# RunhuiWang/DeltaPQ

Hardware: AMD Instinct MI355X
Metric: queries/sec, SIFT1M-shaped m=8 k=256 topk=100 (higher is better)
Workload: dtype f64 sum of f32 table entries (u8 code decode; the reference's incremental f64 stack); 1 GPU

## Files before the change

deltapq_amd/_lib.py:

```python
import ctypes
import os

_HERE = os.path.dirname(os.path.abspath(__file__))
LIB_PATH = os.environ.get("DPQ_LIB_PATH") or os.path.join(_HERE, "csrc", "libdeltapq_amd.so")

c_i32, c_i64, c_f32 = ctypes.c_int32, ctypes.c_int64, ctypes.c_float
P = ctypes.POINTER


class OpenOpts(ctypes.Structure):
    _fields_ = [("device", c_i32), ("shard_rank", c_i32), ("shard_count", c_i32), ("chunks_per_segment", c_i32),
                ("cand_capacity", c_i32), ("num_codes", c_i32), ("bootstrap", c_i32), ("batch_decode", c_i32),
                ("global_offset", c_i64), ("global_n_codes", c_i64),
                ("stream_max_queries", c_i32), ("coarse_below", c_i32), ("plan_ratios", c_i32 * 3), ("boot_cap", c_i32),
                ("boot_target", c_i32), ("flags", c_i32), ("batch_tile_nodes", c_i64)]


class Info(ctypes.Structure):
    _fields_ = [("n_codes_total", c_i64), ("n_bytes_total", c_i64), ("node_lo", c_i64), ("node_hi", c_i64),
                ("algorithmic_bytes", c_i64), ("device_bytes", c_i64), ("n_diffs", c_i64), ("M", c_i32),
                ("K", c_i32), ("Ds", c_i32), ("n_segments", c_i32), ("chunks_per_segment", c_i32),
                ("max_depth", c_i32), ("device", c_i32), ("cand_capacity", c_i32), ("bootstrap_bytes", c_i64),
                ("bootstrap_stride", c_i32), ("batch_decode_mb", c_i32), ("strand_bytes", c_i64)]

# ... 212 lines not shown
    ("dpq_opq_train", ctypes.c_int,
     [_VP, c_i64, ctypes.c_int, ctypes.c_int, ctypes.c_int, P(OpqOpts), _VP, _VP, P(OpqStats)]),
    ("dpq_write_rotation", ctypes.c_int, [ctypes.c_char_p, _VP, ctypes.c_int]),
    ("dpq_read_rotation", ctypes.c_int, [ctypes.c_char_p, P(c_i32), _VP]),
    ("dpq_query_batch_tables", ctypes.c_int, [_VP, _VP, _VP, ctypes.c_int, ctypes.c_int, _VP, _VP]),
    ("dpq_query_batch_device_tables", ctypes.c_int, [_VP, _VP, _VP, ctypes.c_int, ctypes.c_int, _VP, _VP, _VP]),
    ("dpq_range_search_tables", ctypes.c_int, [_VP, _VP, ctypes.c_int, _VP, P(_VP)]),
    ("dpq_ip_tables", ctypes.c_int, [_VP, _VP, ctypes.c_int, _VP, _VP]),
    ("dpq_ip_tables_device", ctypes.c_int, [_VP, _VP, ctypes.c_int, _VP, _VP, _VP]),
    ("dpq_query_batch_ip", ctypes.c_int, [_VP, _VP, _VP, ctypes.c_int, ctypes.c_int, _VP, _VP, _VP, _VP]),
    ("dpq_query_batch_device_ip", ctypes.c_int, [_VP, _VP, _VP, ctypes.c_int, ctypes.c_int, _VP, _VP, _VP, _VP, _VP]),
    ("dpq_ip_scores", ctypes.c_int, [_VP, _VP, _VP, ctypes.c_int, ctypes.c_int, _VP]),
    ("dpq_profile_enable", ctypes.c_int, [_VP, ctypes.c_int]),
    ("dpq_profile_reset", ctypes.c_int, [_VP]),
    ("dpq_profile_read", ctypes.c_int, [_VP, P(Profile)]),
    ("dpq_debug_scan_time", ctypes.c_int, [_VP, ctypes.c_int, ctypes.c_int, ctypes.c_int, ctypes.c_int, P(ctypes.c_float)]),
    ("dpq_debug_scan_stamps", ctypes.c_int, [_VP, ctypes.c_int, ctypes.c_int, P(ctypes.c_ulonglong), ctypes.c_int, P(ctypes.c_float)]),
    ("dpq_debug_boot_stamps", ctypes.c_int, [_VP, ctypes.c_int, P(ctypes.c_double)]),
    ("dpq_debug_select_time", ctypes.c_int, [_VP, ctypes.c_int, ctypes.c_int, ctypes.c_int, ctypes.c_int, P(ctypes.c_float)]),
    ("dpq_debug_strand1_stamps", ctypes.c_int, [_VP, _VP, ctypes.c_int]),
    ("dpq_debug_range_keys", ctypes.c_int, [_VP, P(c_i64)]),
    ("dpq_debug_filter_tables", ctypes.c_int, [_VP, ctypes.c_int, _VP, c_i64]),
    ("dpq_debug_relabel", ctypes.c_int, [_VP, _VP, ctypes.c_int]),
]

_lib = None
_hip_runtime = None


def _bind_hip_runtime():
    global _hip_runtime
    if _hip_runtime is not None:
        return _hip_runtime
    import importlib.util
    candidates = []
    override = os.environ.get("DPQ_HIP_RUNTIME")
    if override:
        candidates.append(override)
    try:
        spec = importlib.util.find_spec("torch")
        if spec is not None and spec.submodule_search_locations:
            candidates.append(os.path.join(list(spec.submodule_search_locations)[0], "lib", "libamdhip64.so"))
    except (ImportError, ValueError):
        pass
    rocm = os.environ.get("ROCM_PATH", "/opt/rocm")
    candidates += [os.path.join(rocm, "lib", "libamdhip64.so"), "libamdhip64.so"]
# ... 43 lines not shown
```

deltapq_amd/csrc/dpq_capi.cpp:

```cpp
#include "dpq_capi_internal.h"

namespace {

thread_local std::string g_last_error;

}

int fail(int code, const std::string& msg) {
    g_last_error = msg;
    return code;
}

uint64_t next_index_serial() {
    static std::atomic<uint64_t> next{1};
    return next++;
}

bool dev_mode() {
    const char* dev = getenv("DPQ_DEV");
    return dev && atoi(dev) != 0;
}

namespace {

// ... 320 lines not shown
int prepare_batch(dpq_index* x, Batch* b) {
    int rc;
    if ((rc = ensure_plan(x, b->top_k, b->cap, b->plan_shape))) return rc;
    int64_t stride = b->top_k;
    for (size_t l = 1; l < x->level_cnt.size(); ++l)
        stride = std::max(stride, regions_for(x, x->level_cnt[l], b->ngroups, b->top_k, b->cap).stride);
    const int s1_region_cap = std::min(std::max(64, b->top_k), 256);
    if (b->strand1) stride = std::max<int64_t>(stride, (int64_t)b->top_k + (int64_t)dpq::kStrand1Regions * s1_region_cap);
    if (stride > INT32_MAX) return fail(DPQ_ERR_NOMEM, "candidate buffer too large");
    if ((rc = ensure_workspace(x, b->nqp, (int)stride))) return rc;
    b->stride = x->ws().cap;
    if (b->scratch && (rc = ensure_batch_raw(x))) return rc;
    return DPQ_OK;
}

int build_tables(dpq_index* x, const Batch& b, const TableSource& src, hipStream_t stream, bool row_stats = true) {
    Workspace& w = x->ws();
    int rc;
    if (b.one_tile && (rc = ensure_plain_image(x, stream))) return rc;
    {
        Timer t(x, stream, 0);
        const uint8_t* relabel = b.scratch ? x->d_relabel.get() : nullptr;
        uint32_t* tight = x->tune.tighten ? w.d_tight.get() : nullptr;
        if (src.d_tables)
            DPQ_HIP(dpq::launch_tables_ingest(src.d_tables, b.nq, b.nqp, x->M, x->K, w.d_lut32, w.d_lut_min, w.d_overflow,
                                              relabel, w.d_lut32r, tight, src.d_bad, stream));
        else
            DPQ_HIP(dpq::launch_lut_build(x->d_codebook, src.d_queries, b.nq, b.nqp, x->M, x->K, x->Ds, w.d_lut32,
                                          w.d_lut_min, nullptr, w.d_overflow, relabel, w.d_lut32r, tight, stream));
        if (row_stats) DPQ_HIP(dpq::launch_row_stats(w.d_lut32, b.nq, x->M, w.d_lut_stat, stream));
    }
    if (x->prof) x->prof_acc.lut_launches++;
    return DPQ_OK;
}

dpq::ScanArgs batch_scan_args(const dpq_index* x, const Batch& b) {
    const Workspace& w = x->ws();
    dpq::ScanArgs sa{};
    sa.img = x->img;
    if (b.one_tile) sa.img.raw = x->d_plain_image;
    sa.fp32_accum = x->plain ? 1 : 0;
    sa.lut32 = b.labelled ? w.d_lut32r.get() : w.d_lut32.get();
    sa.lut_min = w.d_lut_min;
    sa.lut_stat = w.d_lut_stat;
    sa.thr_key = w.d_thr_key;
    sa.slot_query = nullptr;
    sa.n_queries = b.nq;
    sa.cand_count = w.d_cand_count;
    sa.cand_key = w.d_cand_key;
    sa.cand_stride = b.stride;
    sa.region_off = b.top_k;
    sa.counters = x->prof && !x->prof_scan_only ? x->d_counters.get() : nullptr;
    sa.qtab = w.d_qtab;
// ... 1524 lines not shown
```

deltapq_amd/csrc/dpq_capi_debug.cpp:

```cpp
#include "dpq_capi_internal.h"

namespace {

dpq::ScanArgs debug_scan_args(const dpq_index* x, int nq, int* splits) {
    const Workspace& w = x->ws();
    const int QG = dpq::queries_per_group(x->M);
    dpq::ScanArgs sa{};
    sa.img = x->img;
    sa.fp32_accum = x->plain ? 1 : 0;
    sa.lut32 = w.d_lut32;
    sa.lut_min = w.d_lut_min;
    sa.lut_stat = w.d_lut_stat;
    sa.thr_key = w.d_thr_key;
    sa.slot_query = nullptr;
    sa.n_queries = nq;
    sa.seg_list = nullptr;
    sa.n_seg_pass = x->img.n_segments;
    if (const char* e = getenv("DPQ_DEBUG_NSEG")) sa.n_seg_pass = std::min(x->img.n_segments, atoi(e));
    if (*splits <= 0) *splits = splits_for(sa.n_seg_pass, (nq + QG - 1) / QG);
    sa.cand_count = w.d_cand_count;
    sa.cand_key = w.d_cand_key;
    sa.cand_stride = w.cap;
    sa.region_off = 0;
    sa.region_cap = std::max(1, w.cap / *splits);
// ... 225 lines not shown
        sa.lut_min = w.d_lut_min;
        sa.lut_stat = w.d_lut_stat;
        sa.thr_key = w.d_dbg_thr;
        sa.n_queries = w.dbg_qtab_nq;
        DPQ_HIP(dpq::launch_saturation_debug(sa, slots, d_rec, nullptr));
        DPQ_HIP(hipMemcpy(static_cast<char*>(out) + tables, d_rec.get(), records, hipMemcpyDeviceToHost));
    }
    return DPQ_OK;
    });
}

int dpq_debug_relabel(dpq_index* x, unsigned char* out, int bytes) {
    return guarded([&]() -> int {
    DPQ_DEV_ONLY();
    if (!x || !out || bytes < x->M * 256) return fail(DPQ_ERR_ARG, "bad argument");
    if (!x->d_relabel) return fail(DPQ_ERR_STATE, "the handle has no label map");
    DPQ_HIP(hipSetDevice(x->device));
    DPQ_HIP(hipDeviceSynchronize());
    DPQ_HIP(hipMemcpy(out, x->d_relabel.get(), (size_t)x->M * 256, hipMemcpyDeviceToHost));
    return DPQ_OK;
    });
}

int dpq_debug_range_keys(dpq_index* x, int64_t* max_keys) {
    DPQ_DEV_ONLY();
    if (!x || !max_keys) return fail(DPQ_ERR_ARG, "NULL argument");
    *max_keys = x->range.last_max_keys;
    return DPQ_OK;
}

int dpq_debug_select_time(dpq_index* x, int nq, int top_k, int flags, int reps, float* ms_out) {
    return guarded([&]() -> int {
    DPQ_DEV_ONLY();
    if (!x || !ms_out || !x->ws().d_lut32 || !x->d_l0_id) return fail(DPQ_ERR_STATE, "run a query batch first");
    DPQ_HIP(hipSetDevice(x->device));
    const Workspace& w = x->ws();
    dpq::SelectArgs se{};
    se.shared_id = x->d_l0_id;
    se.shared_code = x->d_l0_code;
    se.shared_n = x->l0_segments * dpq::kChunk * x->img.chunks_per_segment;
    se.cand_count = w.d_cand_count;
    se.cand_key = w.d_cand_key;
    se.cand_stride = w.cap;
    se.region_off = top_k;
    se.scratch = w.d_scratch;
    se.lut32 = w.d_lut32;
// ... 25 lines not shown
```

deltapq_amd/csrc/dpq_kernels.h:

```cpp
#pragma once
#include <hip/hip_runtime.h>

#include <cstdint>

#include "dpq_format.h"

#ifndef DPQ_UNDER_SCAN_PRIO
#define DPQ_UNDER_SCAN_PRIO 3
#endif

namespace dpq {

constexpr int kScanThreads = 1024;
constexpr int kScanWaves = kScanThreads / 64;
constexpr int kMaxTopK = 2048;
constexpr int kSelectThreads = 512;
constexpr int kMaxSplits = 256;
constexpr int kRegionStride = 1 + kMaxSplits;
constexpr int kLevel0Nodes = 3840;
constexpr int kSortMax = 4096;
constexpr int queries_per_group(int M) { return M <= 8 ? 64 : 32; }
constexpr int kTightBuckets = 8;
constexpr int kTightSplits = 32;
constexpr int kTightWords = kTightSplits * kTightBuckets / 4;
constexpr int kS1Replicas = 8, kS1ReplicaWords = 512;
constexpr int kS1HistWords = kS1Replicas * kS1ReplicaWords;
static_assert(queries_per_group(8) * kTightWords >= kS1HistWords, "strand1's histogram exceeds what one query group clears");
constexpr int kLutQueries = 8;
constexpr int kLutMinParts = 4;

struct DeviceImage {
    const uint8_t* nib = nullptr;
    const uint8_t* par = nullptr;
    const uint8_t* carry = nullptr;
    const uint8_t* mask = nullptr;
    const uint8_t* delta = nullptr;
    const uint64_t* seg_delta_off = nullptr;
    const uint8_t* seg_ckpt = nullptr;
    const uint8_t* raw = nullptr;
    const uint64_t* st_ckpt = nullptr;
    const uint32_t* st_mask = nullptr;
    const uint16_t* st_depth = nullptr;
    const uint32_t* st_pbase = nullptr;
    const uint8_t* st_delta = nullptr;
    int32_t n_strips = 0;
    int64_t n_local = 0;
    int64_t n_codes_total = 0;
    uint32_t id_base = 0;
    int32_t n_segments = 0;
    int32_t chunks_per_segment = 4;
    int32_t M = 8, K = 256;
};
// ... 90 lines not shown
    const int32_t* slot_query;
    const uint32_t* cand_count;
    int32_t n_slots, n_regions, n_queries;
    uint32_t* max_count;
    int64_t* lims;
};

struct RangeEmitArgs {
    const int64_t* out_off;
    const uint32_t* cand_count;
    const uint64_t* cand_key;
    int64_t cand_stride;
    int32_t region_off, region_cap, n_regions;
    int32_t lds_keys;
    int32_t* out_ids;
    float* out_dists;
    int64_t out_n;
    uint64_t* scratch;
    int64_t n_codes_total;
};

hipError_t launch_lut_build(const float* d_codebook, const float* d_queries, int nq, int n_slots, int M, int K, int Ds,
                            float* d_lut32, float* d_lut_min, uint32_t* d_cand_count, uint32_t* d_overflow,
                            const uint8_t* d_relabel, float* d_lut_labels, uint32_t* d_tight_hist,
                            hipStream_t stream);
hipError_t launch_decode_list(const DeviceImage& img, const uint32_t* seg_list, int n_seg, const uint8_t* relabel,
                              uint32_t* out_code, hipStream_t stream);
hipError_t launch_decode_segments(const DeviceImage& img, const uint32_t* seg_list, int n_seg, uint32_t* out_id,
                                  uint32_t* out_code, hipStream_t stream);
hipError_t launch_stream(const ScanArgs& a, int n_slots, hipStream_t stream);
hipError_t launch_strand(const ScanArgs& a, int n_slots, hipStream_t stream);
int stream_queries_per_pass(int M, int n_slots);
hipError_t launch_strand1(const ScanArgs& a, int n_slots, hipStream_t stream);
int strand1_workgroups(int n_strips);
constexpr int kStrand1Regions = 256;
hipError_t launch_quantise(const ScanArgs& a, int n_slot_groups, hipStream_t stream);
hipError_t launch_row_stats(const float* d_lut32, int nq, int M, float* d_lut_stat, hipStream_t stream);
hipError_t launch_scan(const ScanArgs& a, int n_slot_groups, int splits, hipStream_t stream);
size_t qtab_bytes_per_group(int M);
hipError_t launch_saturation_debug(const ScanArgs& a, int n_slots, unsigned char* d_out, hipStream_t stream);
int scan_stamp_count();
hipError_t launch_select(const SelectArgs& a, int M, int n_slots, hipStream_t stream);
hipError_t launch_bootstrap(const BootArgs& a, int M, int n_slots, hipStream_t stream);
hipError_t launch_range_count(const RangeCountArgs& a, hipStream_t stream);
hipError_t launch_range_emit(const RangeEmitArgs& a, int n_slots, hipStream_t stream);
hipError_t launch_merge(const int32_t* d_ids, const float* d_dists, int n_lists, int nq, int top_k, int row_stride,
                        int32_t* d_out_ids, float* d_out_dists, hipStream_t stream);
// ... 7 lines not shown
```

deltapq_amd/csrc/dpq_kernels.hip:

```cpp
#include "dpq_kernels.h"
#include "dpq_wave_decoder.h"

#include <atomic>
#include <type_traits>
#include <cfloat>
#include <cmath>

namespace dpq {

static hipError_t ensure_dynamic_lds(const void* fn, size_t bytes, std::atomic<bool>* done);


__device__ __forceinline__ uint32_t and_or(uint32_t a, uint32_t mask, uint32_t c) {
    uint32_t r;
    asm("v_and_or_b32 %0, %1, %2, %3" : "=v"(r) : "v"(a), "s"(mask), "v"(c));
    return r;
}

__device__ __forceinline__ uint64_t make_key(float d, uint32_t id) {
    return ((uint64_t)__float_as_uint(d) << 32) | (uint64_t)id;
}

__device__ __forceinline__ float lut_min_of(const float* __restrict__ lut_min, size_t q, int M, int m) {
    const float4 p = *reinterpret_cast<const float4*>(lut_min + (q * M + m) * kLutMinParts);
    return fminf(fminf(p.x, p.y), fminf(p.z, p.w));
}

__global__ __launch_bounds__(256) void lut_build_kernel(const float* __restrict__ codebook,
                                                         const float* __restrict__ queries, int nq, int n_slots, int M,
                                                         int K, int Ds, float* __restrict__ lut,
                                                         float* __restrict__ lut_min, uint32_t* __restrict__ cand_count,
                                                         uint32_t* __restrict__ overflow, const uint8_t* __restrict__ relabel,
                                                         float* __restrict__ lut_labels, uint32_t* __restrict__ tight_hist) {
    __builtin_amdgcn_s_setprio(DPQ_UNDER_SCAN_PRIO);
    const int q0 = blockIdx.x * kLutQueries, m = blockIdx.y, k = threadIdx.x;
    if (m == 0 && k < kLutQueries && q0 + k < n_slots) {
        if (cand_count) cand_count[q0 + k] = 0;
        if (overflow) overflow[q0 + k] = 0;
    }
    if (m == 0 && tight_hist)
        for (int i = k; i < kLutQueries * kTightWords; i += 256)
            if (q0 * kTightWords + i < n_slots * kTightWords) tight_hist[(size_t)q0 * kTightWords + i] = 0;
    if (q0 >= nq) return;
    float acc[kLutQueries];
#pragma unroll
    for (int j = 0; j < kLutQueries; ++j) acc[j] = 0.0f;
    if (k < K) {
        const float* c = codebook + ((size_t)m * K + k) * Ds;
        const float* qv = queries + (size_t)q0 * M * Ds + (size_t)m * Ds;
        const size_t qstride = (size_t)M * Ds;
        auto step = [&](float& a, float cv, float qd) {
            const float diff = __fsub_rn(cv, qd);
            const double sq = __dmul_rn((double)diff, (double)diff);
            a = (float)__dadd_rn((double)a, sq);
        };
        if ((Ds & 3) == 0) {
            const float4* c4 = reinterpret_cast<const float4*>(c);
            for (int d = 0; d < Ds; d += 4) {
                const float4 v = c4[d >> 2];
#pragma unroll
                for (int j = 0; j < kLutQueries; ++j) {
                    const float* qj = qv + (size_t)min(j, nq - 1 - q0) * qstride + d;
                    step(acc[j], v.x, qj[0]);
                    step(acc[j], v.y, qj[1]);
                    step(acc[j], v.z, qj[2]);
                    step(acc[j], v.w, qj[3]);
                }
            }
        } else {
            for (int d = 0; d < Ds; ++d) {
                const float cv = c[d];
#pragma unroll
                for (int j = 0; j < kLutQueries; ++j) step(acc[j], cv, qv[(size_t)min(j, nq - 1 - q0) * qstride + d]);
            }
        }
    } else {
#pragma unroll
        for (int j = 0; j < kLutQueries; ++j) acc[j] = INFINITY;
    }
#pragma unroll
    for (int j = 0; j < kLutQueries; ++j) {
        if (q0 + j < nq) lut[((size_t)(q0 + j) * M + m) * 256 + k] = acc[j];
        if (lut_labels && q0 + j < nq) lut_labels[((size_t)(q0 + j) * M + m) * 256 + relabel[m * 256 + k]] = acc[j];
        uint32_t v = __float_as_uint(acc[j]);
#pragma unroll
        for (int o = 32; o > 0; o >>= 1) v = min(v, (uint32_t)__shfl_xor((int)v, o));
        if ((k & 63) == 0 && q0 + j < nq) lut_min[((size_t)(q0 + j) * M + m) * kLutMinParts + (k >> 6)] = __uint_as_float(v);
    }
}

template <int M>
__global__ __launch_bounds__(64) void decode_segments_kernel(const DeviceImage img,
                                                              const uint32_t* __restrict__ seg_list,
                                                              uint32_t* __restrict__ out_id,
                                                              uint32_t* __restrict__ out_code) {
    constexpr int W = Cfg<M>::W;
    const int lane = threadIdx.x;
    const uint32_t seg = seg_list ? seg_list[blockIdx.x] : blockIdx.x;
    const int cps = img.chunks_per_segment;
    WaveDecoder<M> dec;
    if (!img.raw) dec.begin_segment(img, seg, lane);
    for (int c = 0; c < cps; ++c) {
        const int64_t node = ((int64_t)seg * cps + c) * 64 + lane;
        uint32_t code[W];
        if (img.raw) {
#pragma unroll
            for (int w = 0; w < W; ++w) code[w] = reinterpret_cast<const uint32_t*>(img.raw)[(size_t)node * W + w];
        } else {
            dec.step(img, node, lane, c + 1 < cps, code);
        }
// ... 79 lines not shown
        }
    }
    return r;
}

template <int M>
__device__ __forceinline__ float filter_offset(const FilterScale& fs, float min_m, int m) {
    const float mn = fs.s32 != 0.0f ? min_m : 0.0f;
    const double od = (double)mn * (double)fs.s32;
    float of = (float)od;
    if ((double)of < od) of = __uint_as_float(__float_as_uint(of) + 1u);
    const double sd = (m == 0 ? (double)fs.bias : 0.0) - 0.5 - (double)of;
    float sf = (float)sd;
    if ((double)sf > sd) sf = __uint_as_float(__float_as_uint(sf) + (sf > 0.0f ? -1 : 1));
    return sf;
}

template <int M>
__device__ __forceinline__ uint32_t filter_field(float tv, float sc, float of, uint32_t clamp) {
    const float fv = fminf(__fmaf_rn(tv, sc, of), (float)clamp);
    return __builtin_amdgcn_cvt_pk_u8_f32(fv, 0u, 0u);
}

constexpr int kSatRank = 32;

template <int M>
__global__ __launch_bounds__(64 * M) void row_stat_kernel(const float* __restrict__ lut32, float* __restrict__ lut_stat) {
    const int q = blockIdx.x, m = threadIdx.x >> 6, lane = threadIdx.x & 63;
    const float* row = lut32 + ((size_t)q * M + m) * 256;
    uint32_t x[4];
#pragma unroll
    for (int j = 0; j < 4; ++j) x[j] = __float_as_uint(row[lane + 64 * j]) & 0x7fffffffu;
    uint32_t r = 0;
    for (int b = 30; b >= 0; --b) {
        const uint32_t c = r | (1u << b);
        int n = 0;
#pragma unroll
        for (int j = 0; j < 4; ++j) n += __popcll(__ballot(x[j] >= c));
        if (n >= kSatRank) r = c;
    }
    if (lane == 0) lut_stat[(size_t)q * M + m] = __uint_as_float(r);
}

template <int M>
__device__ __forceinline__ uint32_t filter_row_stat(float entry, float sc, float of) {
    return (uint32_t)fmaxf(fminf(__fmaf_rn(entry, sc, of), (float)Cfg<M>::SAT_CAP), 0.0f);
}

template <int M>
__device__ __forceinline__ int filter_saturations(uint32_t stat_m, int lane) {
    using C = Cfg<M>;
    static_assert(M == 8, "groups of eight lanes");
    constexpr int CAP = C::SAT_CAP;
    auto sum8 = [](int v) {
        v += __builtin_amdgcn_update_dpp(0, v, 0xB1, 0xf, 0xf, true);
        v += __builtin_amdgcn_update_dpp(0, v, 0x4E, 0xf, 0xf, true);
        v += __builtin_amdgcn_update_dpp(0, v, 0x141, 0xf, 0xf, true);
        return v;
    };
    const int stat = (int)stat_m;
    const bool uniform = sum8(stat) == 0;
    bool open = true;
    int sat = 0, rem = C::SAT_BUDGET, num = 0, den = 1;
    for (int it = 0; it < M && __ballot(open) != 0; ++it) {
// ... 2430 lines not shown
    const size_t lds = ((size_t)K * Ds + (size_t)Ds * 256) * sizeof(float);
    if (lds > 160 * 1024) return hipErrorInvalidValue;
    static std::atomic<bool> done[64] = {};
    hipError_t e = ensure_dynamic_lds(reinterpret_cast<const void*>(&encode_pq_kernel), 160 * 1024, done);
    if (e != hipSuccess) return e;
    hipLaunchKernelGGL(encode_pq_kernel, dim3((unsigned)((n + 255) / 256), (unsigned)M), dim3(256), lds, stream,
                       d_vectors, n, D, d_codebook, M, K, Ds, d_codes);
    return hipGetLastError();
}

size_t scan_lds_bytes(int M) { return M <= 8 ? ScanLds<8>::kBytes : ScanLds<16>::kBytes; }

size_t select_lds_bytes(int M, int top_k, int n_shared) {
    size_t kp = 1;
    while (kp < (size_t)top_k) kp <<= 1;
    const size_t n_keys = n_shared > 0 ? (size_t)std::min(n_shared, kSortMax) : (size_t)select_list_keys(top_k);
    const size_t area = n_shared > 0 ? kp : (size_t)select_area_keys(top_k);
    const size_t select_bytes = area * 8 + 266 * 4, table_bytes = n_shared > 0 ? (size_t)M * 256 * 4 : 0;
    return n_keys * 8 + std::max(select_bytes, table_bytes) + 16;
}

hipError_t launch_lut_build(const float* d_codebook, const float* d_queries, int nq, int n_slots, int M, int K, int Ds,
                            float* d_lut32, float* d_lut_min, uint32_t* d_cand_count, uint32_t* d_overflow,
                            const uint8_t* d_relabel, float* d_lut_labels, uint32_t* d_tight_hist, hipStream_t stream) {
    if (nq <= 0) return hipSuccess;
    n_slots = std::max(n_slots, nq);
    hipLaunchKernelGGL(lut_build_kernel, dim3((unsigned)((n_slots + kLutQueries - 1) / kLutQueries), (unsigned)M),
                       dim3(256), 0, stream, d_codebook, d_queries, nq, n_slots, M, K, Ds, d_lut32, d_lut_min,
                       d_cand_count, d_overflow, d_relabel, d_relabel ? d_lut_labels : nullptr, d_tight_hist);
    return hipGetLastError();
}

hipError_t launch_decode_segments(const DeviceImage& img, const uint32_t* seg_list, int n_seg, uint32_t* out_id,
                                  uint32_t* out_code, hipStream_t stream) {
    if (n_seg <= 0) return hipSuccess;
    if (img.M == 8)
        hipLaunchKernelGGL(decode_segments_kernel<8>, dim3((unsigned)n_seg), dim3(64), 0, stream, img, seg_list,
                           out_id, out_code);
    else if (img.M == 16)
        hipLaunchKernelGGL(decode_segments_kernel<16>, dim3((unsigned)n_seg), dim3(64), 0, stream, img, seg_list,
                           out_id, out_code);
    else
        return hipErrorInvalidValue;
    return hipGetLastError();
}

hipError_t launch_decode_list(const DeviceImage& img, const uint32_t* seg_list, int n_seg, const uint8_t* relabel,
                              uint32_t* out_code, hipStream_t stream) {
    if (n_seg <= 0) return hipSuccess;
    const unsigned grid = (unsigned)((n_seg + 3) / 4);
    if (img.M == 8)
        hipLaunchKernelGGL(decode_list_kernel<8>, dim3(grid), dim3(256), 0, stream, img, seg_list, n_seg, relabel, out_code);
// ... 220 lines not shown
```

deltapq_amd/csrc/dpq_tables.h:

```cpp
#pragma once
#include <hip/hip_runtime.h>

#include <cstdint>

namespace dpq {

constexpr int kIpQueries = 4;

hipError_t launch_tables_ingest(const float* d_tables, int nq, int n_slots, int M, int K, float* d_lut32, float* d_lut_min,
                                uint32_t* d_overflow, const uint8_t* d_relabel, float* d_lut_labels, uint32_t* d_tight_hist,
                                uint32_t* d_bad, hipStream_t stream);

hipError_t launch_ip_tables(const float* d_codebook, const float* d_queries, int nq, int M, int K, int Ds, float* d_tables,
                            float* d_bias, hipStream_t stream);

hipError_t launch_ip_scores(const float* d_bias, const float* d_gaps, const int32_t* d_ids, int nq, int top_k,
                            float* d_scores, hipStream_t stream);

}
```

deltapq_amd/csrc/dpq_tables.hip:

```cpp
#include "dpq_tables.h"

#include <algorithm>
#include <cmath>

#include "dpq_kernels.h"

namespace dpq {

__global__ __launch_bounds__(256) void tables_ingest_kernel(const float* __restrict__ tables, int nq, int n_slots, int M,
                                                             int K, float* __restrict__ lut, float* __restrict__ lut_min,
                                                             uint32_t* __restrict__ overflow,
                                                             const uint8_t* __restrict__ relabel,
                                                             float* __restrict__ lut_labels,
                                                             uint32_t* __restrict__ tight_hist, uint32_t* __restrict__ bad) {
    __builtin_amdgcn_s_setprio(DPQ_UNDER_SCAN_PRIO);
    const int q = blockIdx.x, m = blockIdx.y, k = threadIdx.x;
    if (m == 0) {
        if (k == 0 && overflow) overflow[q] = 0;
        if (tight_hist)
            for (int i = k; i < kTightWords; i += 256) tight_hist[(size_t)q * kTightWords + i] = 0;
    }
    if (q >= nq) return;
    float v = INFINITY;
    if (k < K) {
        v = tables[((size_t)q * M + m) * K + k];
        if (!(v >= 0.0f)) {
            v = INFINITY;
            *bad = 1u;
        }
    }
    uint32_t b = __float_as_uint(v);
    if (b == 0x80000000u) b = 0u;
    v = __uint_as_float(b);
    lut[((size_t)q * M + m) * 256 + k] = v;
    if (lut_labels) lut_labels[((size_t)q * M + m) * 256 + relabel[m * 256 + k]] = v;
#pragma unroll
    for (int o = 32; o > 0; o >>= 1) b = min(b, (uint32_t)__shfl_xor((int)b, o));
    if ((k & 63) == 0) lut_min[((size_t)q * M + m) * kLutMinParts + (k >> 6)] = __uint_as_float(b);
}

__global__ __launch_bounds__(256) void ip_tables_kernel(const float* __restrict__ codebook, const float* __restrict__ queries,
                                                         int nq, int M, int K, int Ds, float* __restrict__ tables,
                                                         float* __restrict__ bias) {
    __shared__ float wave_top[4][kIpQueries];
    const int q0 = blockIdx.x * kIpQueries, k = threadIdx.x;
    const int nj = min(kIpQueries, nq - q0);
    const size_t qstride = (size_t)M * Ds;
    double B[kIpQueries];
#pragma unroll
    for (int j = 0; j < kIpQueries; ++j) B[j] = 0.0;
    for (int m = 0; m < M; ++m) {
        double acc[kIpQueries];
#pragma unroll
        for (int j = 0; j < kIpQueries; ++j) acc[j] = 0.0;
        if (k < K) {
            const float* c = codebook + ((size_t)m * K + k) * Ds;
            const float* qv = queries + (size_t)q0 * qstride + (size_t)m * Ds;
            for (int d = 0; d < Ds; ++d) {
                const double cv = (double)c[d];
#pragma unroll
                for (int j = 0; j < kIpQueries; ++j)
// ... 15 lines not shown
            const float top = fmaxf(fmaxf(wave_top[0][j], wave_top[1][j]), fmaxf(wave_top[2][j], wave_top[3][j]));
            B[j] = __dadd_rn(B[j], (double)top);
            if (k < K && j < nj) tables[((size_t)(q0 + j) * M + m) * K + k] = __fsub_rn(top, p[j]);
        }
        __syncthreads();
    }
    if (k == 0) {
#pragma unroll
        for (int j = 0; j < kIpQueries; ++j)
            if (j < nj) bias[q0 + j] = (float)B[j];
    }
}

__global__ __launch_bounds__(256) void ip_scores_kernel(const float* __restrict__ bias, const float* __restrict__ gaps,
                                                         const int32_t* __restrict__ ids, int top_k, int64_t n,
                                                         float* __restrict__ scores) {
    const int64_t i = (int64_t)blockIdx.x * 256 + threadIdx.x;
    if (i >= n) return;
    scores[i] = ids[i] < 0 ? -INFINITY : (float)__dsub_rn((double)bias[i / top_k], (double)gaps[i]);
}

hipError_t launch_tables_ingest(const float* d_tables, int nq, int n_slots, int M, int K, float* d_lut32, float* d_lut_min,
                                uint32_t* d_overflow, const uint8_t* d_relabel, float* d_lut_labels, uint32_t* d_tight_hist,
                                uint32_t* d_bad, hipStream_t stream) {
    if (nq <= 0) return hipSuccess;
    n_slots = std::max(n_slots, nq);
    hipLaunchKernelGGL(tables_ingest_kernel, dim3((unsigned)n_slots, (unsigned)M), dim3(256), 0, stream, d_tables, nq, n_slots,
                       M, K, d_lut32, d_lut_min, d_overflow, d_relabel, d_relabel ? d_lut_labels : nullptr, d_tight_hist,
                       d_bad);
    return hipGetLastError();
}

hipError_t launch_ip_tables(const float* d_codebook, const float* d_queries, int nq, int M, int K, int Ds, float* d_tables,
                            float* d_bias, hipStream_t stream) {
    if (nq <= 0) return hipSuccess;
    hipLaunchKernelGGL(ip_tables_kernel, dim3((unsigned)((nq + kIpQueries - 1) / kIpQueries)), dim3(256), 0, stream,
                       d_codebook, d_queries, nq, M, K, Ds, d_tables, d_bias);
    return hipGetLastError();
}

hipError_t launch_ip_scores(const float* d_bias, const float* d_gaps, const int32_t* d_ids, int nq, int top_k,
                            float* d_scores, hipStream_t stream) {
    const int64_t n = (int64_t)nq * top_k;
    if (n <= 0) return hipSuccess;
    hipLaunchKernelGGL(ip_scores_kernel, dim3((unsigned)((n + 255) / 256)), dim3(256), 0, stream, d_bias, d_gaps, d_ids,
                       top_k, n, d_scores);
    return hipGetLastError();
}

}
```

include/deltapq_amd.h:

```cpp
#ifndef DELTAPQ_AMD_H
#define DELTAPQ_AMD_H

#include <stdint.h>

#ifdef __cplusplus
extern "C" {
#endif

#define DPQ_VERSION 100

typedef enum dpq_status {
    DPQ_OK = 0,
    DPQ_ERR_ARG = -1,
    DPQ_ERR_IO = -2,
    DPQ_ERR_FORMAT = -3,
    DPQ_ERR_NO_DEVICE = -4,
    DPQ_ERR_HIP = -5,
    DPQ_ERR_NOMEM = -6,
    DPQ_ERR_STATE = -7,
    DPQ_ERR_TOPK = -8
} dpq_status;

typedef struct dpq_index dpq_index;
typedef struct dpq_soa dpq_soa;
// ... 398 lines not shown
                                  int32_t* d_ids, float* d_dists, void* hip_stream);
int dpq_range_search_tables(dpq_index* idx, const float* tables, int nq, const float* radii, dpq_range_result** out);

int dpq_ip_tables(dpq_index* idx, const float* queries, int nq, float* tables_out, float* bias_out);
int dpq_ip_tables_device(dpq_index* idx, const float* d_queries, int nq, float* d_tables, float* d_bias, void* hip_stream);
int dpq_query_batch_ip(dpq_index* idx, const dpq_filter* filter, const float* queries, int nq, int top_k, int32_t* ids,
                       float* scores, float* gaps_out, float* bias_out);
int dpq_query_batch_device_ip(dpq_index* idx, const dpq_filter* filter, const float* d_queries, int nq, int top_k,
                              int32_t* d_ids, float* d_scores, float* d_gaps, float* d_bias, void* hip_stream);
int dpq_ip_scores(const float* bias, const float* gaps, const int32_t* ids, int nq, int top_k, float* scores_out);

int dpq_profile_enable(dpq_index* idx, int on);
int dpq_profile_reset(dpq_index* idx);
int dpq_profile_read(dpq_index* idx, dpq_profile* out);

int dpq_debug_scan_time(dpq_index* idx, int nq, int pass_all, int reps, int splits, float* ms_out);
int dpq_debug_scan_stamps(dpq_index* idx, int nq, int splits, unsigned long long* out, int n_out, float* ms_out);
int dpq_debug_boot_stamps(dpq_index* idx, int nq, double* out);
int dpq_debug_select_time(dpq_index* idx, int nq, int top_k, int flags, int reps, float* ms_out);
int dpq_debug_range_keys(dpq_index* idx, int64_t* max_keys);
int dpq_debug_strand1_stamps(dpq_index* idx, unsigned long long* out, int n_words);
int dpq_debug_filter_tables(dpq_index* idx, int lane, void* out, int64_t bytes);
int dpq_debug_relabel(dpq_index* idx, unsigned char* out, int bytes);

#ifdef __cplusplus
}
#endif
#endif
```

Baseline: 6.778 million queries/s.

## Fuse row-stat rank into LUT build and ingest kernels with wave-wide rows

Removes the separate row_stats kernel launch by computing the saturation-rank statistic inside the LUT build and table-ingest kernels. Both kernels move from 256-thread blocks to a single 64-lane wave that holds four table entries per lane, and the LUT build now handles four queries per block. The rank search is rewritten with inline compare and popcount assembly, and lut_min now stores the whole-row minimum in all four parts. The fused stat is only computed when M==8, so other M values no longer get lut_stat filled. A debug entry point for checking table builds is also added.

```diff
diff --git a/deltapq_amd/_lib.py b/deltapq_amd/_lib.py
--- a/deltapq_amd/_lib.py
+++ b/deltapq_amd/_lib.py
@@ -258,6 +258,8 @@
     ("dpq_debug_range_keys", ctypes.c_int, [_VP, P(c_i64)]),
     ("dpq_debug_filter_tables", ctypes.c_int, [_VP, ctypes.c_int, _VP, c_i64]),
     ("dpq_debug_relabel", ctypes.c_int, [_VP, _VP, ctypes.c_int]),
+    ("dpq_debug_table_build", ctypes.c_int,
+     [_VP, _VP, _VP, ctypes.c_int, ctypes.c_int, _VP, _VP, _VP, _VP, _VP, _VP, _VP]),
 ]
 
 _lib = None
diff --git a/deltapq_amd/csrc/dpq_capi.cpp b/deltapq_amd/csrc/dpq_capi.cpp
--- a/deltapq_amd/csrc/dpq_capi.cpp
+++ b/deltapq_amd/csrc/dpq_capi.cpp
@@ -366,13 +366,13 @@
         Timer t(x, stream, 0);
         const uint8_t* relabel = b.scratch ? x->d_relabel.get() : nullptr;
         uint32_t* tight = x->tune.tighten ? w.d_tight.get() : nullptr;
+        float* stat = row_stats ? w.d_lut_stat.get() : nullptr;
         if (src.d_tables)
             DPQ_HIP(dpq::launch_tables_ingest(src.d_tables, b.nq, b.nqp, x->M, x->K, w.d_lut32, w.d_lut_min, w.d_overflow,
-                                              relabel, w.d_lut32r, tight, src.d_bad, stream));
+                                              relabel, w.d_lut32r, tight, src.d_bad, stat, stream));
         else
             DPQ_HIP(dpq::launch_lut_build(x->d_codebook, src.d_queries, b.nq, b.nqp, x->M, x->K, x->Ds, w.d_lut32,
-                                          w.d_lut_min, nullptr, w.d_overflow, relabel, w.d_lut32r, tight, stream));
-        if (row_stats) DPQ_HIP(dpq::launch_row_stats(w.d_lut32, b.nq, x->M, w.d_lut_stat, stream));
+                                          w.d_lut_min, nullptr, w.d_overflow, relabel, w.d_lut32r, tight, stat, stream));
     }
     if (x->prof) x->prof_acc.lut_launches++;
     return DPQ_OK;
diff --git a/deltapq_amd/csrc/dpq_capi_debug.cpp b/deltapq_amd/csrc/dpq_capi_debug.cpp
--- a/deltapq_amd/csrc/dpq_capi_debug.cpp
+++ b/deltapq_amd/csrc/dpq_capi_debug.cpp
@@ -271,6 +271,54 @@
     });
 }
 
+int dpq_debug_table_build(dpq_index* x, const float* queries, const float* tables, int nq, int n_slots, float* lut32,
+                          float* lut_labels, float* lut_min, float* lut_stat, uint32_t* cand_count, uint32_t* overflow,
+                          uint32_t* tight) {
+    return guarded([&]() -> int {
+    DPQ_DEV_ONLY();
+    if (!x || (!queries && !tables) || nq <= 0 || n_slots < nq || n_slots > kMaxBatchQueries || !lut32 || !lut_min ||
+        !lut_stat || !cand_count || !overflow || !tight)
+        return fail(DPQ_ERR_ARG, "bad argument");
+    if (!tables && !x->d_codebook) return fail(DPQ_ERR_STATE, "the handle has no codebook");
+    if (lut_labels && !x->d_relabel) return fail(DPQ_ERR_STATE, "the handle has no label map");
+    DPQ_HIP(hipSetDevice(x->device));
+    const size_t rows = (size_t)n_slots * x->M;
+    const size_t n_in = tables ? (size_t)nq * x->M * x->K : (size_t)nq * x->M * x->Ds;
+    DevBuf<float> d_in, d_lut, d_lab, d_min, d_stat;
+    DevBuf<uint32_t> d_cnt, d_over, d_tight, d_bad;
+    int rc;
+    if ((rc = d_in.alloc(n_in)) || (rc = d_lut.alloc(rows * 256)) || (rc = d_lab.alloc(rows * 256)) ||
+        (rc = d_min.alloc(rows * dpq::kLutMinParts)) || (rc = d_stat.alloc(rows)) || (rc = d_cnt.alloc((size_t)n_slots)) ||
+        (rc = d_over.alloc((size_t)n_slots)) || (rc = d_tight.alloc((size_t)n_slots * dpq::kTightWords)) || (rc = d_bad.alloc(1)))
+        return rc;
+    DPQ_HIP(hipMemcpy(d_in, tables ? tables : queries, sizeof(float) * n_in, hipMemcpyHostToDevice));
+    DPQ_HIP(hipMemset(d_lut, 0xff, sizeof(float) * rows * 256));
+    DPQ_HIP(hipMemset(d_lab, 0xff, sizeof(float) * rows * 256));
+    DPQ_HIP(hipMemset(d_min, 0xff, sizeof(float) * rows * dpq::kLutMinParts));
+    DPQ_HIP(hipMemset(d_stat, 0xff, sizeof(float) * rows));
+    DPQ_HIP(hipMemset(d_cnt, 0xff, sizeof(uint32_t) * n_slots));
+    DPQ_HIP(hipMemset(d_over, 0xff, sizeof(uint32_t) * n_slots));
+    DPQ_HIP(hipMemset(d_tight, 0xff, sizeof(uint32_t) * n_slots * dpq::kTightWords));
+    DPQ_HIP(hipMemset(d_bad, 0, sizeof(uint32_t)));
+    const uint8_t* relabel = lut_labels ? x->d_relabel.get() : nullptr;
+    if (tables)
+        DPQ_HIP(dpq::launch_tables_ingest(d_in, nq, n_slots, x->M, x->K, d_lut, d_min, d_over, relabel, d_lab, d_tight, d_bad,
+                                          d_stat, nullptr));
+    else
+        DPQ_HIP(dpq::launch_lut_build(x->d_codebook, d_in, nq, n_slots, x->M, x->K, x->Ds, d_lut, d_min, d_cnt, d_over,
+                                      relabel, d_lab, d_tight, d_stat, nullptr));
+    DPQ_HIP(hipDeviceSynchronize());
+    DPQ_HIP(hipMemcpy(lut32, d_lut, sizeof(float) * rows * 256, hipMemcpyDeviceToHost));
+    if (lut_labels) DPQ_HIP(hipMemcpy(lut_labels, d_lab, sizeof(float) * rows * 256, hipMemcpyDeviceToHost));
+    DPQ_HIP(hipMemcpy(lut_min, d_min, sizeof(float) * rows * dpq::kLutMinParts, hipMemcpyDeviceToHost));
+    DPQ_HIP(hipMemcpy(lut_stat, d_stat, sizeof(float) * rows, hipMemcpyDeviceToHost));
+    DPQ_HIP(hipMemcpy(cand_count, d_cnt, sizeof(uint32_t) * n_slots, hipMemcpyDeviceToHost));
+    DPQ_HIP(hipMemcpy(overflow, d_over, sizeof(uint32_t) * n_slots, hipMemcpyDeviceToHost));
+    DPQ_HIP(hipMemcpy(tight, d_tight, sizeof(uint32_t) * n_slots * dpq::kTightWords, hipMemcpyDeviceToHost));
+    return DPQ_OK;
+    });
+}
+
 int dpq_debug_range_keys(dpq_index* x, int64_t* max_keys) {
     DPQ_DEV_ONLY();
     if (!x || !max_keys) return fail(DPQ_ERR_ARG, "NULL argument");
diff --git a/deltapq_amd/csrc/dpq_kernels.h b/deltapq_amd/csrc/dpq_kernels.h
--- a/deltapq_amd/csrc/dpq_kernels.h
+++ b/deltapq_amd/csrc/dpq_kernels.h
@@ -26,8 +26,54 @@
 constexpr int kS1Replicas = 8, kS1ReplicaWords = 512;
 constexpr int kS1HistWords = kS1Replicas * kS1ReplicaWords;
 static_assert(queries_per_group(8) * kTightWords >= kS1HistWords, "strand1's histogram exceeds what one query group clears");
-constexpr int kLutQueries = 8;
+constexpr int kLutQueries = 4;
+constexpr int kLutRowRegs = 4;
 constexpr int kLutMinParts = 4;
+constexpr int kSatRank = 32;
+
+#ifdef __HIP__
+__device__ __forceinline__ uint32_t row_min_bits(const uint32_t (&x)[kLutRowRegs]) {
+    uint32_t v = min(min(x[0], x[1]), min(x[2], x[3]));
+#pragma unroll
+    for (int o = 32; o > 0; o >>= 1) v = min(v, (uint32_t)__shfl_xor((int)v, o));
+    return v;
+}
+template <int N>
+__device__ __forceinline__ void row_rank_bits(const uint32_t (&x)[N][kLutRowRegs], uint32_t (&r)[N]) {
+    uint32_t y[N][kLutRowRegs];
+#pragma unroll
+    for (int j = 0; j < N; ++j) {
+        r[j] = 0;
+#pragma unroll
+        for (int i = 0; i < kLutRowRegs; ++i) y[j][i] = x[j][i] & 0x7fffffffu;
+    }
+    static_assert(kLutRowRegs == 4, "the count below compares four registers");
+    for (int b = 30; b >= 0; --b) {
+#pragma unroll
+        for (int j = 0; j < N; ++j) {
+            const uint32_t c = r[j] | (1u << b);
+            uint64_t m0, m1, m2, m3;
+            uint32_t n, n1, n2, n3;
+            asm("v_cmp_ge_u32_e64 %[m0], %[y0], %[c]\n\t"
+                "v_cmp_ge_u32_e64 %[m1], %[y1], %[c]\n\t"
+                "v_cmp_ge_u32_e64 %[m2], %[y2], %[c]\n\t"
+                "v_cmp_ge_u32_e64 %[m3], %[y3], %[c]\n\t"
+                "s_bcnt1_i32_b64 %[n], %[m0]\n\t"
+                "s_bcnt1_i32_b64 %[n1], %[m1]\n\t"
+                "s_bcnt1_i32_b64 %[n2], %[m2]\n\t"
+                "s_bcnt1_i32_b64 %[n3], %[m3]\n\t"
+                "s_add_i32 %[n], %[n], %[n1]\n\t"
+                "s_add_i32 %[n2], %[n2], %[n3]\n\t"
+                "s_add_i32 %[n], %[n], %[n2]"
+                : [n] "=&s"(n), [n1] "=&s"(n1), [n2] "=&s"(n2), [n3] "=&s"(n3), [m0] "=&s"(m0), [m1] "=&s"(m1),
+                  [m2] "=&s"(m2), [m3] "=&s"(m3)
+                : [y0] "v"(y[j][0]), [y1] "v"(y[j][1]), [y2] "v"(y[j][2]), [y3] "v"(y[j][3]), [c] "s"(c)
+                : "scc");
+            if (n >= (uint32_t)kSatRank) r[j] = c;
+        }
+    }
+}
+#endif
 
 struct DeviceImage {
     const uint8_t* nib = nullptr;
@@ -164,7 +210,7 @@
 
 hipError_t launch_lut_build(const float* d_codebook, const float* d_queries, int nq, int n_slots, int M, int K, int Ds,
                             float* d_lut32, float* d_lut_min, uint32_t* d_cand_count, uint32_t* d_overflow,
-                            const uint8_t* d_relabel, float* d_lut_labels, uint32_t* d_tight_hist,
+                            const uint8_t* d_relabel, float* d_lut_labels, uint32_t* d_tight_hist, float* d_lut_stat,
                             hipStream_t stream);
 hipError_t launch_decode_list(const DeviceImage& img, const uint32_t* seg_list, int n_seg, const uint8_t* relabel,
                               uint32_t* out_code, hipStream_t stream);
diff --git a/deltapq_amd/csrc/dpq_kernels.hip b/deltapq_amd/csrc/dpq_kernels.hip
--- a/deltapq_amd/csrc/dpq_kernels.hip
+++ b/deltapq_amd/csrc/dpq_kernels.hip
@@ -26,66 +26,100 @@
     return fminf(fminf(p.x, p.y), fminf(p.z, p.w));
 }
 
-__global__ __launch_bounds__(256) void lut_build_kernel(const float* __restrict__ codebook,
-                                                         const float* __restrict__ queries, int nq, int n_slots, int M,
-                                                         int K, int Ds, float* __restrict__ lut,
-                                                         float* __restrict__ lut_min, uint32_t* __restrict__ cand_count,
-                                                         uint32_t* __restrict__ overflow, const uint8_t* __restrict__ relabel,
-                                                         float* __restrict__ lut_labels, uint32_t* __restrict__ tight_hist) {
+__global__ __launch_bounds__(64) void lut_build_kernel(const float* __restrict__ codebook,
+                                                        const float* __restrict__ queries, int nq, int n_slots, int M,
+                                                        int K, int Ds, float* __restrict__ lut,
+                                                        float* __restrict__ lut_min, uint32_t* __restrict__ cand_count,
+                                                        uint32_t* __restrict__ overflow, const uint8_t* __restrict__ relabel,
+                                                        float* __restrict__ lut_labels, uint32_t* __restrict__ tight_hist,
+                                                        float* __restrict__ lut_stat) {
     __builtin_amdgcn_s_setprio(DPQ_UNDER_SCAN_PRIO);
-    const int q0 = blockIdx.x * kLutQueries, m = blockIdx.y, k = threadIdx.x;
-    if (m == 0 && k < kLutQueries && q0 + k < n_slots) {
-        if (cand_count) cand_count[q0 + k] = 0;
-        if (overflow) overflow[q0 + k] = 0;
-    }
-    if (m == 0 && tight_hist)
-        for (int i = k; i < kLutQueries * kTightWords; i += 256)
-            if (q0 * kTightWords + i < n_slots * kTightWords) tight_hist[(size_t)q0 * kTightWords + i] = 0;
+    constexpr int R = kLutRowRegs;
+    const int q0 = blockIdx.x * kLutQueries, m = blockIdx.y, lane = threadIdx.x;
+    if (m == 0) {
+        if (lane < kLutQueries && q0 + lane < n_slots) {
+            if (cand_count) cand_count[q0 + lane] = 0;
+            if (overflow) overflow[q0 + lane] = 0;
+        }
+        if (tight_hist)
+            for (int i = lane; i < kLutQueries * kTightWords; i += 64)
+                if (q0 * kTightWords + i < n_slots * kTightWords) tight_hist[(size_t)q0 * kTightWords + i] = 0;
+    }
     if (q0 >= nq) return;
-    float acc[kLutQueries];
-#pragma unroll
-    for (int j = 0; j < kLutQueries; ++j) acc[j] = 0.0f;
-    if (k < K) {
-        const float* c = codebook + ((size_t)m * K + k) * Ds;
-        const float* qv = queries + (size_t)q0 * M * Ds + (size_t)m * Ds;
-        const size_t qstride = (size_t)M * Ds;
-        auto step = [&](float& a, float cv, float qd) {
-            const float diff = __fsub_rn(cv, qd);
-            const double sq = __dmul_rn((double)diff, (double)diff);
-            a = (float)__dadd_rn((double)a, sq);
-        };
-        if ((Ds & 3) == 0) {
-            const float4* c4 = reinterpret_cast<const float4*>(c);
-            for (int d = 0; d < Ds; d += 4) {
-                const float4 v = c4[d >> 2];
-#pragma unroll
-                for (int j = 0; j < kLutQueries; ++j) {
-                    const float* qj = qv + (size_t)min(j, nq - 1 - q0) * qstride + d;
-                    step(acc[j], v.x, qj[0]);
-                    step(acc[j], v.y, qj[1]);
-                    step(acc[j], v.z, qj[2]);
-                    step(acc[j], v.w, qj[3]);
-                }
-            }
-        } else {
-            for (int d = 0; d < Ds; ++d) {
-                const float cv = c[d];
-#pragma unroll
-                for (int j = 0; j < kLutQueries; ++j) step(acc[j], cv, qv[(size_t)min(j, nq - 1 - q0) * qstride + d]);
+    float acc[kLutQueries][R];
+#pragma unroll
+    for (int j = 0; j < kLutQueries; ++j)
+#pragma unroll
+        for (int r = 0; r < R; ++r) acc[j][r] = 0.0f;
+    const float* c[R];
+#pragma unroll
+    for (int r = 0; r < R; ++r) c[r] = codebook + ((size_t)m * K + min(lane + 64 * r, K - 1)) * Ds;
+    const float* qv = queries + (size_t)q0 * M * Ds + (size_t)m * Ds;
+    const size_t qstride = (size_t)M * Ds;
+    const int jmax = nq - 1 - q0;
+    auto step = [&](float& a, float cv, float qd) {
+        const float diff = __fsub_rn(cv, qd);
+        a = (float)__fma_rn((double)diff, (double)diff, (double)a);
+    };
+    if ((Ds & 3) == 0) {
+        for (int d = 0; d < Ds; d += 4) {
+            float4 v[R];
+#pragma unroll
+            for (int r = 0; r < R; ++r) v[r] = reinterpret_cast<const float4*>(c[r])[d >> 2];
+#pragma unroll
+            for (int j = 0; j < kLutQueries; ++j) {
+                const float* qj = qv + (size_t)min(j, jmax) * qstride + d;
+                const float q0d = qj[0], q1d = qj[1], q2d = qj[2], q3d = qj[3];
+#pragma unroll
+                for (int r = 0; r < R; ++r) {
+                    step(acc[j][r], v[r].x, q0d);
+                    step(acc[j][r], v[r].y, q1d);
+                    step(acc[j][r], v[r].z, q2d);
+                    step(acc[j][r], v[r].w, q3d);
+                }
             }
         }
     } else {
-#pragma unroll
-        for (int j = 0; j < kLutQueries; ++j) acc[j] = INFINITY;
-    }
+        for (int d = 0; d < Ds; ++d) {
+            float cv[R];
+#pragma unroll
+            for (int r = 0; r < R; ++r) cv[r] = c[r][d];
+#pragma unroll
+            for (int j = 0; j < kLutQueries; ++j) {
+                const float qd = qv[(size_t)min(j, jmax) * qstride + d];
+#pragma unroll
+                for (int r = 0; r < R; ++r) step(acc[j][r], cv[r], qd);
+            }
+        }
+    }
+    uint32_t x[kLutQueries][R];
+#pragma unroll
+    for (int j = 0; j < kLutQueries; ++j)
+#pragma unroll
+        for (int r = 0; r < R; ++r) x[j][r] = lane + 64 * r < K ? __float_as_uint(acc[j][r]) : 0x7f800000u;
+    int label[R];
+#pragma unroll
+    for (int r = 0; r < R; ++r) label[r] = lut_labels ? relabel[m * 256 + lane + 64 * r] : 0;
 #pragma unroll
     for (int j = 0; j < kLutQueries; ++j) {
-        if (q0 + j < nq) lut[((size_t)(q0 + j) * M + m) * 256 + k] = acc[j];
-        if (lut_labels && q0 + j < nq) lut_labels[((size_t)(q0 + j) * M + m) * 256 + relabel[m * 256 + k]] = acc[j];
-        uint32_t v = __float_as_uint(acc[j]);
-#pragma unroll
-        for (int o = 32; o > 0; o >>= 1) v = min(v, (uint32_t)__shfl_xor((int)v, o));
-        if ((k & 63) == 0 && q0 + j < nq) lut_min[((size_t)(q0 + j) * M + m) * kLutMinParts + (k >> 6)] = __uint_as_float(v);
+        if (q0 + j >= nq) break;
+        const size_t row = ((size_t)(q0 + j) * M + m) * 256;
+#pragma unroll
+        for (int r = 0; r < R; ++r) lut[row + lane + 64 * r] = __uint_as_float(x[j][r]);
+        if (lut_labels) {
+#pragma unroll
+            for (int r = 0; r < R; ++r) lut_labels[row + label[r]] = __uint_as_float(x[j][r]);
+        }
+        const float mn = __uint_as_float(row_min_bits(x[j]));
+        if (lane == 0)
+            *reinterpret_cast<float4*>(lut_min + ((size_t)(q0 + j) * M + m) * kLutMinParts) = make_float4(mn, mn, mn, mn);
+    }
+    if (lut_stat) {
+        uint32_t st[kLutQueries];
+        row_rank_bits<kLutQueries>(x, st);
+#pragma unroll
+        for (int j = 0; j < kLutQueries; ++j)
+            if (lane == 0 && q0 + j < nq) lut_stat[(size_t)(q0 + j) * M + m] = __uint_as_float(st[j]);
     }
 }
 
@@ -211,24 +245,16 @@
     return __builtin_amdgcn_cvt_pk_u8_f32(fv, 0u, 0u);
 }
 
-constexpr int kSatRank = 32;
 
 template <int M>
 __global__ __launch_bounds__(64 * M) void row_stat_kernel(const float* __restrict__ lut32, float* __restrict__ lut_stat) {
     const int q = blockIdx.x, m = threadIdx.x >> 6, lane = threadIdx.x & 63;
     const float* row = lut32 + ((size_t)q * M + m) * 256;
-    uint32_t x[4];
-#pragma unroll
-    for (int j = 0; j < 4; ++j) x[j] = __float_as_uint(row[lane + 64 * j]) & 0x7fffffffu;
-    uint32_t r = 0;
-    for (int b = 30; b >= 0; --b) {
-        const uint32_t c = r | (1u << b);
-        int n = 0;
-#pragma unroll
-        for (int j = 0; j < 4; ++j) n += __popcll(__ballot(x[j] >= c));
-        if (n >= kSatRank) r = c;
-    }
-    if (lane == 0) lut_stat[(size_t)q * M + m] = __uint_as_float(r);
+    uint32_t x[1][kLutRowRegs], r[1];
+#pragma unroll
+    for (int j = 0; j < kLutRowRegs; ++j) x[0][j] = __float_as_uint(row[lane + 64 * j]);
+    row_rank_bits<1>(x, r);
+    if (lane == 0) lut_stat[(size_t)q * M + m] = __uint_as_float(r[0]);
 }
 
 template <int M>
@@ -2705,12 +2731,15 @@
 
 hipError_t launch_lut_build(const float* d_codebook, const float* d_queries, int nq, int n_slots, int M, int K, int Ds,
                             float* d_lut32, float* d_lut_min, uint32_t* d_cand_count, uint32_t* d_overflow,
-                            const uint8_t* d_relabel, float* d_lut_labels, uint32_t* d_tight_hist, hipStream_t stream) {
+                            const uint8_t* d_relabel, float* d_lut_labels, uint32_t* d_tight_hist, float* d_lut_stat,
+                            hipStream_t stream) {
     if (nq <= 0) return hipSuccess;
+    if (K < 1 || K > 256) return hipErrorInvalidValue;
     n_slots = std::max(n_slots, nq);
     hipLaunchKernelGGL(lut_build_kernel, dim3((unsigned)((n_slots + kLutQueries - 1) / kLutQueries), (unsigned)M),
-                       dim3(256), 0, stream, d_codebook, d_queries, nq, n_slots, M, K, Ds, d_lut32, d_lut_min,
-                       d_cand_count, d_overflow, d_relabel, d_relabel ? d_lut_labels : nullptr, d_tight_hist);
+                       dim3(64), 0, stream, d_codebook, d_queries, nq, n_slots, M, K, Ds, d_lut32, d_lut_min,
+                       d_cand_count, d_overflow, d_relabel, d_relabel ? d_lut_labels : nullptr, d_tight_hist,
+                       M == 8 ? d_lut_stat : nullptr);
     return hipGetLastError();
 }
 
diff --git a/deltapq_amd/csrc/dpq_tables.h b/deltapq_amd/csrc/dpq_tables.h
--- a/deltapq_amd/csrc/dpq_tables.h
+++ b/deltapq_amd/csrc/dpq_tables.h
@@ -9,7 +9,7 @@
 
 hipError_t launch_tables_ingest(const float* d_tables, int nq, int n_slots, int M, int K, float* d_lut32, float* d_lut_min,
                                 uint32_t* d_overflow, const uint8_t* d_relabel, float* d_lut_labels, uint32_t* d_tight_hist,
-                                uint32_t* d_bad, hipStream_t stream);
+                                uint32_t* d_bad, float* d_lut_stat, hipStream_t stream);
 
 hipError_t launch_ip_tables(const float* d_codebook, const float* d_queries, int nq, int M, int K, int Ds, float* d_tables,
                             float* d_bias, hipStream_t stream);
diff --git a/deltapq_amd/csrc/dpq_tables.hip b/deltapq_amd/csrc/dpq_tables.hip
--- a/deltapq_amd/csrc/dpq_tables.hip
+++ b/deltapq_amd/csrc/dpq_tables.hip
@@ -7,36 +7,47 @@
 
 namespace dpq {
 
-__global__ __launch_bounds__(256) void tables_ingest_kernel(const float* __restrict__ tables, int nq, int n_slots, int M,
-                                                             int K, float* __restrict__ lut, float* __restrict__ lut_min,
-                                                             uint32_t* __restrict__ overflow,
-                                                             const uint8_t* __restrict__ relabel,
-                                                             float* __restrict__ lut_labels,
-                                                             uint32_t* __restrict__ tight_hist, uint32_t* __restrict__ bad) {
+__global__ __launch_bounds__(64) void tables_ingest_kernel(const float* __restrict__ tables, int nq, int n_slots, int M,
+                                                            int K, float* __restrict__ lut, float* __restrict__ lut_min,
+                                                            uint32_t* __restrict__ overflow,
+                                                            const uint8_t* __restrict__ relabel,
+                                                            float* __restrict__ lut_labels,
+                                                            uint32_t* __restrict__ tight_hist, uint32_t* __restrict__ bad,
+                                                            float* __restrict__ lut_stat) {
     __builtin_amdgcn_s_setprio(DPQ_UNDER_SCAN_PRIO);
-    const int q = blockIdx.x, m = blockIdx.y, k = threadIdx.x;
+    const int q = blockIdx.x, m = blockIdx.y, lane = threadIdx.x;
     if (m == 0) {
-        if (k == 0 && overflow) overflow[q] = 0;
+        if (lane == 0 && overflow) overflow[q] = 0;
         if (tight_hist)
-            for (int i = k; i < kTightWords; i += 256) tight_hist[(size_t)q * kTightWords + i] = 0;
+            for (int i = lane; i < kTightWords; i += 64) tight_hist[(size_t)q * kTightWords + i] = 0;
     }
     if (q >= nq) return;
-    float v = INFINITY;
-    if (k < K) {
-        v = tables[((size_t)q * M + m) * K + k];
-        if (!(v >= 0.0f)) {
-            v = INFINITY;
-            *bad = 1u;
+    const size_t row = ((size_t)q * M + m) * 256;
+    uint32_t x[1][kLutRowRegs];
+#pragma unroll
+    for (int r = 0; r < kLutRowRegs; ++r) {
+        const int k = lane + 64 * r;
+        float v = INFINITY;
+        if (k < K) {
+            v = tables[((size_t)q * M + m) * K + k];
+            if (!(v >= 0.0f)) {
+                v = INFINITY;
+                *bad = 1u;
+            }
         }
+        uint32_t b = __float_as_uint(v);
+        if (b == 0x80000000u) b = 0u;
+        x[0][r] = b;
+        lut[row + k] = __uint_as_float(b);
+        if (lut_labels) lut_labels[row + relabel[m * 256 + k]] = __uint_as_float(b);
     }
-    uint32_t b = __float_as_uint(v);
-    if (b == 0x80000000u) b = 0u;
-    v = __uint_as_float(b);
-    lut[((size_t)q * M + m) * 256 + k] = v;
-    if (lut_labels) lut_labels[((size_t)q * M + m) * 256 + relabel[m * 256 + k]] = v;
-#pragma unroll
-    for (int o = 32; o > 0; o >>= 1) b = min(b, (uint32_t)__shfl_xor((int)b, o));
-    if ((k & 63) == 0) lut_min[((size_t)q * M + m) * kLutMinParts + (k >> 6)] = __uint_as_float(b);
+    const float mn = __uint_as_float(row_min_bits(x[0]));
+    if (lane == 0) *reinterpret_cast<float4*>(lut_min + ((size_t)q * M + m) * kLutMinParts) = make_float4(mn, mn, mn, mn);
+    if (lut_stat) {
+        uint32_t st[1];
+        row_rank_bits<1>(x, st);
+        if (lane == 0) lut_stat[(size_t)q * M + m] = __uint_as_float(st[0]);
+    }
 }
 
 __global__ __launch_bounds__(256) void ip_tables_kernel(const float* __restrict__ codebook, const float* __restrict__ queries,
@@ -98,12 +109,13 @@
 
 hipError_t launch_tables_ingest(const float* d_tables, int nq, int n_slots, int M, int K, float* d_lut32, float* d_lut_min,
                                 uint32_t* d_overflow, const uint8_t* d_relabel, float* d_lut_labels, uint32_t* d_tight_hist,
-                                uint32_t* d_bad, hipStream_t stream) {
+                                uint32_t* d_bad, float* d_lut_stat, hipStream_t stream) {
     if (nq <= 0) return hipSuccess;
+    if (K < 1 || K > 256) return hipErrorInvalidValue;
     n_slots = std::max(n_slots, nq);
-    hipLaunchKernelGGL(tables_ingest_kernel, dim3((unsigned)n_slots, (unsigned)M), dim3(256), 0, stream, d_tables, nq, n_slots,
+    hipLaunchKernelGGL(tables_ingest_kernel, dim3((unsigned)n_slots, (unsigned)M), dim3(64), 0, stream, d_tables, nq, n_slots,
                        M, K, d_lut32, d_lut_min, d_overflow, d_relabel, d_relabel ? d_lut_labels : nullptr, d_tight_hist,
-                       d_bad);
+                       d_bad, M == 8 ? d_lut_stat : nullptr);
     return hipGetLastError();
 }
 
diff --git a/include/deltapq_amd.h b/include/deltapq_amd.h
--- a/include/deltapq_amd.h
+++ b/include/deltapq_amd.h
@@ -444,6 +444,9 @@
 int dpq_debug_strand1_stamps(dpq_index* idx, unsigned long long* out, int n_words);
 int dpq_debug_filter_tables(dpq_index* idx, int lane, void* out, int64_t bytes);
 int dpq_debug_relabel(dpq_index* idx, unsigned char* out, int bytes);
+int dpq_debug_table_build(dpq_index* idx, const float* queries, const float* tables, int nq, int n_slots, float* lut32,
+                          float* lut_labels, float* lut_min, float* lut_stat, uint32_t* cand_count, uint32_t* overflow,
+                          uint32_t* tight);
 
 #ifdef __cplusplus
 }
```

Result: no change. 6.736 million queries/s (median of 2 runs) (-0.6%).
